# jenkinsm13/julia-spira

Hardware: AMD Instinct MI355X
Metric: Msamples/sec at 1920x1080 spp=64 depth=8; fraction of HBM roofline (higher is better)
Workload: dtype f64

## Files before the change

### julia-spira_amd/csrc/spira_device.h

```cpp
#pragma once
#include <hip/hip_runtime.h>
#include <stdint.h>
#include <type_traits>
#include "spira_fastdiv.h"

namespace spira {

__device__ __forceinline__ float sqrt_rn(float x) { return __builtin_sqrtf(x); }
__device__ __forceinline__ double sqrt_rn(double x) { return __builtin_sqrt(x); }

constexpr int kBlock = 256;
#ifndef SPIRA_WAVES_F32
#define SPIRA_WAVES_F32 5
#endif
#ifndef SPIRA_WAVES_F64
#define SPIRA_WAVES_F64 4
#endif
#define SPIRA_WAVES_PER_SIMD(T) (sizeof(T) == 8 ? SPIRA_WAVES_F64 : SPIRA_WAVES_F32)
constexpr uint32_t kMaxTries = 64;

template <class T> struct Vec { T x, y, z; };

template <class T> __device__ __forceinline__ Vec<T> mk(T x, T y, T z) { Vec<T> r; r.x = x; r.y = y; r.z = z; return r; }
template <class T> __device__ __forceinline__ Vec<T> operator+(Vec<T> a, Vec<T> b) { return mk<T>(a.x + b.x, a.y + b.y, a.z + b.z); }
// ... 1168 lines not shown
        a.blk_stats[4 * wid + 1] = n_rmw;
        a.blk_stats[4 * wid + 2] = n_store;
        a.blk_stats[4 * wid + 3] = FIRST ? 0u : n_seg;
    }
}

template <class T> struct PathArgs {
    SceneGlobal<T> scene;
    RenderConst<T> rc;
    RayQueue<T> q[2];
    uint32_t *qref[2];
    uint2 *qkey[2];
    uint32_t cam_consts;
    Pack3<T> *L;
    uint32_t *blk_stats;
    uint32_t cap;
    uint32_t pass;
    uint32_t n_first;
    uint32_t dense_pct;
    Pack4<T> *mesh_list;
    uint32_t mesh_min_batch;
    uint32_t refill_free;
    uint32_t mesh_mode;
    uint32_t *mesh_count;
    uint32_t resume_k, resume_nw;
    uint32_t *redo;
    uint32_t redo_only;
    Stats *stats;
    Pack4<T> *accum;
    FastDiv fd_keff;
    uint32_t k_eff;
    uint32_t accum_first;
    uint32_t l_private;
};

#ifndef SPIRA_RESOLVE_RUN
#define SPIRA_RESOLVE_RUN 4
#endif
__device__ __forceinline__ uint32_t owned_pixel(uint32_t w, uint32_t nw, uint32_t l) {
    constexpr uint32_t kRun = SPIRA_RESOLVE_RUN;
    static_assert(64 % kRun == 0, "a run length divides the wave");
    return ((l / kRun) * nw + w) * kRun + l % kRun;
}

template <class T>
__device__ __forceinline__ void resolve_pixel(Pack4<T> *accum, const Pack3<T> *L, uint32_t tile_pixels, uint32_t k_eff, bool first_pass, uint32_t p) {
    Pack4<T> acc;
    if (first_pass) { acc.x = 0; acc.y = 0; acc.z = 0; acc.w = 0; } else acc = accum[p];
    uint32_t s = 0;
    for (; s + 8 <= k_eff; s += 8) {
        Pack3<T> l[8];
#pragma unroll
        for (int k = 0; k < 8; ++k) l[k] = L[(size_t)(s + k) * tile_pixels + p];
#pragma unroll
        for (int k = 0; k < 8; ++k) { acc.x = acc.x + l[k].x; acc.y = acc.y + l[k].y; acc.z = acc.z + l[k].z; }
    }
    for (; s < k_eff; ++s) {
        const Pack3<T> l = L[(size_t)s * tile_pixels + p];
        acc.x = acc.x + l.x; acc.y = acc.y + l.y; acc.z = acc.z + l.z;
    }
    accum[p] = acc;
}
template <class T>
__device__ __forceinline__ void resolve_pixel_run(Pack4<T> *accum, const Pack3<T> *Lp, uint32_t k_eff, bool first_pass, uint32_t p) {
    constexpr uint32_t kRun = SPIRA_RESOLVE_RUN;
    Pack4<T> acc;
    if (first_pass) { acc.x = 0; acc.y = 0; acc.z = 0; acc.w = 0; } else acc = accum[p];
    uint32_t s = 0;
    for (; s + 8 <= k_eff; s += 8) {
        Pack3<T> l[8];
#pragma unroll
        for (int k = 0; k < 8; ++k) l[k] = Lp[(s + k) * kRun];
#pragma unroll
        for (int k = 0; k < 8; ++k) { acc.x = acc.x + l[k].x; acc.y = acc.y + l[k].y; acc.z = acc.z + l[k].z; }
    }
    for (; s < k_eff; ++s) {
        const Pack3<T> l = Lp[s * kRun];
        acc.x = acc.x + l.x; acc.y = acc.y + l.y; acc.z = acc.z + l.z;
    }
    accum[p] = acc;
}

__device__ __forceinline__ float pack_qref(uint32_t q, uint32_t, float) { return __uint_as_float(q); }
__device__ __forceinline__ double pack_qref(uint32_t q, uint32_t ref, double) { return __longlong_as_double((long long)((unsigned long long)q | ((unsigned long long)ref << 32))); }
__device__ __forceinline__ uint32_t unpack_q(float w) { return __float_as_uint(w); }
__device__ __forceinline__ uint32_t unpack_q(double w) { return (uint32_t)(unsigned long long)__double_as_longlong(w); }
__device__ __forceinline__ uint32_t unpack_ref(double w) { return (uint32_t)((unsigned long long)__double_as_longlong(w) >> 32); }

#ifdef SPIRA_MESH_STATS
__device__ unsigned long long g_mesh_dbg[32];
#define MESH_STAT(...) __VA_ARGS__
#else
#define MESH_STAT(...)
#endif

#ifndef SPIRA_CARRY_KEY
#define SPIRA_CARRY_KEY 1
#endif
#ifndef SPIRA_WAVES_B_F32
#define SPIRA_WAVES_B_F32 4
#endif
#ifndef SPIRA_WAVES_B_F64
#define SPIRA_WAVES_B_F64 SPIRA_WAVES_F64
#endif
#ifndef SPIRA_WAVES_PATH_F32
#define SPIRA_WAVES_PATH_F32 6
#endif
template <class T, int R, bool BVH, bool EXT, bool SPEC, int MODE = 0, bool TRI = true>
__global__ __launch_bounds__(kBlock, MODE == 2 ? (sizeof(T) == 8 ? SPIRA_WAVES_B_F64 : SPIRA_WAVES_B_F32) : (sizeof(T) == 4 ? SPIRA_WAVES_PATH_F32 : SPIRA_WAVES_F64)) void k_path(const PathArgs<T> a) {
    extern __shared__ __attribute__((aligned(32))) unsigned char lds_raw[];
    constexpr uint32_t WPB = kBlock / 64, SUB = 64 * R;
    constexpr bool kRefArray = sizeof(T) == 4;
    constexpr bool kCarry = SPIRA_CARRY_KEY && !BVH && !EXT;
    constexpr uint32_t kStageShift = 25, kRefMask = (1u << kStageShift) - 1u;
    const uint32_t lane = threadIdx.x & 63, wave = threadIdx.x >> 6;
    const uint32_t NW = gridDim.x * WPB, wid = blockIdx.x * WPB + wave;
    const RenderConst<T> &rc = a.rc;
    using Pol = typename std::conditional<SPEC, SpecDiv, ExactDiv>::type;
    Pol pol;
    if (!SPEC && a.redo_only) {
        uint32_t any = 0;
        for (uint32_t w = 0; w < WPB; ++w) any |= a.redo[blockIdx.x * WPB + w];
        if (!any) return;
    }
    T *cam_lds = reinterpret_cast<T *>(lds_raw + scene_lds_bytes<T>(a.scene.n_spheres, a.scene.n_materials, a.scene.n_triangles) + WPB * SUB * sizeof(Pack4<T>));
    if (threadIdx.x < 12) {
        const Vec<T> *cv = threadIdx.x < 3 ? &rc.cam_origin : (threadIdx.x < 6 ? &rc.cam_llc : (threadIdx.x < 9 ? &rc.cam_hor : &rc.cam_ver));
        const uint32_t cc = threadIdx.x % 3;
        cam_lds[threadIdx.x] = cc == 0 ? cv->x : (cc == 1 ? cv->y : cv->z);
    }
    Pack4<T> *cam_sph = reinterpret_cast<Pack4<T> *>(reinterpret_cast<unsigned char *>(cam_lds) + 128);
    constexpr bool kCam = !EXT;
    if (kCam && MODE != 2 && a.cam_consts)
        for (uint32_t i = threadIdx.x; i < a.scene.n_spheres; i += blockDim.x) {
            const T *sp = a.scene.spheres5 + 5 * (size_t)i;
            const Vec<T> oc = rc.cam_origin - mk<T>(sp[0], sp[1], sp[2]);
            Pack4<T> k; k.x = oc.x; k.y = oc.y; k.z = oc.z; k.w = dot(oc, oc) - sp[3] * sp[3];
            cam_sph[i] = k;
        }
    const SceneLds<T> sc = stage_scene<T>(a.scene, lds_raw);
    const PixelDiv<T> pix_div = pixel_divisors<T>(rc);
    if (!SPEC && a.redo_only) {
        if (!a.redo[wid]) return;
        if (lane == 0) atomicAdd(&a.stats->redone_waves, 1ull);
    }
    Pack4<T> *s_rnd = reinterpret_cast<Pack4<T> *>(lds_raw + scene_lds_bytes<T>(a.scene.n_spheres, a.scene.n_materials, a.scene.n_triangles)) + wave * SUB;
    constexpr uint32_t mesh_mode = BVH ? (uint32_t)MODE : 0u;
    const uint32_t kseg = mesh_mode == 2u ? a.resume_k : 1u;
    if (mesh_mode == 2u && wid * kseg >= a.resume_nw) return;
    const uint32_t region = wid * kseg * a.cap;
    const unsigned long long lt_mask = (1ull << lane) - 1ull;
    const uint32_t ref_base = sc.n_spheres + sc.n_triangles;
    const bool mixed = mesh_mode != 0u || rc.max_depth <= 128u;
    const uint32_t dense_pct = mixed ? a.dense_pct : 0u;
    const bool defer = mesh_mode != 0u || (BVH && mixed && a.mesh_list != nullptr);
    Pack4<T> *mlist = a.mesh_list + 3 * (size_t)region;
    uint32_t n_rmw = 0, n_store = 0, n_seg = 0, n_enq = 0, n_park = 0;
    uint32_t n_wtrips = 0, n_ltrips = 0;
    uint32_t n_in = 0;
    const bool own = !BVH && !EXT && !TRI && sizeof(T) == 8 && a.accum != nullptr;
    const uint32_t n_own = own ? 64u * a.k_eff : 0u;
    const uint32_t n_sub_first = own ? (n_own + SUB - 1) / SUB : (a.n_first + SUB - 1) / SUB;
    const bool priv = kCarry && own && a.l_private != 0;
    const uint32_t l_base = priv ? wid * n_own : 0u;

    auto park = [&](uint32_t slot_i, const Vec<T> o_, const Vec<T> d_, const Vec<T> beta_, T closest_, uint32_t q_, int prim_, uint32_t stage_hit) {
        Pack4<T> A, B, C;
        A.x = o_.x; A.y = o_.y; A.z = o_.z; A.w = d_.x;
        B.x = d_.y; B.y = d_.z; B.z = beta_.x; B.w = beta_.y;
        C.x = beta_.z; C.y = closest_; C.z = Bits<T>::from_u32(q_); C.w = Bits<T>::from_u32((uint32_t)(prim_ + 1) | (stage_hit << kStageShift));
        mlist[3 * (size_t)slot_i] = A; mlist[3 * (size_t)slot_i + 1] = B; mlist[3 * (size_t)slot_i + 2] = C;
    };
    uint32_t mfill = 0;
    constexpr int kMaxSeg = 16;
    uint32_t pfx[kMaxSeg + 1];
    bool segmented = false;
    {
        uint32_t cnt = 0;
        if (mesh_mode == 2u && lane < kseg && wid * kseg + lane < a.resume_nw) cnt = a.mesh_count[wid * kseg + lane];
        pfx[0] = 0;
#pragma unroll
        for (int j = 0; j < kMaxSeg; ++j) pfx[j + 1] = pfx[j] + (uint32_t)__builtin_amdgcn_readlane((int)cnt, j);
        if (mesh_mode == 2u) { mfill = pfx[kMaxSeg]; segmented = true; }
    }
    const uint32_t first_sub = own ? 0u : (mesh_mode == 1u ? (wid % a.resume_k) * (NW / a.resume_k) + wid / a.resume_k : wid);
    const uint32_t sub_step = own ? 1u : NW;
    MESH_STAT(unsigned long long dbg_t0 = __builtin_readcyclecounter(); unsigned long long dbg_sess = 0, dbg_walk = 0; uint32_t dbg_ns = 0, dbg_ws = 0, dbg_ls = 0, dbg_rf = 0, dbg_rays = 0, dbg_rounds = 0, dbg_ws1 = 0, dbg_ls1 = 0, dbg_h[4] = {0, 0, 0, 0};)
    for (uint32_t round = 0; ; ++round) {
        MESH_STAT(++dbg_rounds;)
        const bool first = mesh_mode != 2u && round == 0;
        const RayQueue<T> qin = a.q[(round + 1) & 1], qout = a.q[round & 1];
        const uint32_t *rin = a.qref[(round + 1) & 1];
        uint32_t *rout = a.qref[round & 1];
        const uint2 *kin = a.qkey[(round + 1) & 1];
        uint2 *kout = a.qkey[round & 1];
        const uint32_t limit = first ? (own ? n_own : a.n_first) : n_in;
        const uint32_t n_sub = first ? n_sub_first : (n_in + SUB - 1) / SUB;
        uint32_t fill = 0;
        for (uint32_t sub = first ? first_sub : 0u; sub < n_sub; sub += first ? sub_step : 1u) {
            Vec<T> o[R], beta[R];
            Pending<T> pend[R];
            ExtState<T> ex[R];
            uint32_t q[R], ent[R], stg[R], ref[R];
            uint32_t ka[R], kb[R];
            bool valid[R];
#pragma unroll
            for (int r = 0; r < R; ++r) {
                const uint32_t idx = sub * SUB + r * 64 + lane;
                valid[r] = false; stg[r] = round; ref[r] = 0; q[r] = 0; ka[r] = 0; kb[r] = 0;
                pend[r].kind = kDead; pend[r].rough = 0; pend[r].v = mk<T>(0, 0, 0);
                o[r] = mk<T>(0, 0, 0); beta[r] = mk<T>(1, 1, 1);
                bool parked = false; T park_t = 0; int park_prim = -1;
                uint32_t qf = idx;
                bool in = idx < limit;
                if (own && first) {
                    const uint32_t t = idx / SPIRA_RESOLVE_RUN, run = fastdiv(t, a.fd_keff);
                    const uint32_t px = owned_pixel(wid, NW, run * SPIRA_RESOLVE_RUN + idx % SPIRA_RESOLVE_RUN);
                    qf = (t - run * a.k_eff) * rc.tile_pixels + px;
                    in = in && px < rc.tile_pixels;
                }
                const uint32_t ql = priv ? l_base + idx : qf;
                if (in) {
                    if (first) {
                        uint32_t pixel, sample, pi, pj;
                        Vec<T> d;
                        q[r] = ql;
                        path_of<T>(rc, qf, a.pass, pi, pj, pixel, sample);
                        if (kCarry) { ka[r] = mix32(rc.sA + pixel) ^ (sample << 8); kb[r] = mix32(rc.sB ^ pixel) + (sample << 8); }
                        camera_ray_lds<T>(rc, cam_lds, pix_div, pi, pj, pixel, sample, o[r], d, pol);
                        if (EXT) { ex[r].flags = rc.flags; if (rc.flags & kExtSpectral) beta[r] = ext_wavelength<T>(sc, rc.sA, rc.sB, pixel, sample, ex[r]); }
                        T t; uint32_t slot = 0;
                        int prim;
                        if (defer) {
                            if (kCam && a.cam_consts) closest_hit_local<T, Pol, TRI, true>(sc, o[r], d, (T)0.001, t, prim, pol, cam_sph);
                            else closest_hit_local<T, Pol, TRI>(sc, o[r], d, (T)0.001, t, prim, pol);
                            parked = mesh_box_hit<T>(sc, o[r], d, t);
                        } else if (kCam && !BVH && a.cam_consts) { closest_hit_local<T, Pol, TRI, true>(sc, o[r], d, (T)0.001, t, prim, pol, cam_sph); }
                        else prim = closest_hit<T, BVH, Pol, TRI>(sc, o[r], d, (T)0.001, t, slot, pol);
                        ++n_seg;
                        if (parked) { park_t = t; park_prim = prim; pend[r].v = d; }
                        else if (prim < 0) {
                            const Vec<T> c = sky_term_x<T, EXT>(d, beta[r], &ex[r]);
                            Pack3<T> l; l.x = c.x; l.y = c.y; l.z = c.z;
                            a.L[ql] = l;
                            ++n_store;
                        } else {
                            valid[r] = true;
                            o[r] = o[r] + d * t;
                            ref[r] = (BVH && prim >= (int)ref_base) ? ref_base + slot : (uint32_t)prim;
                            pend[r].v = d;
                        }
                    } else {
                        const Pack4<T> A = qin.A[region + idx], B = qin.B[region + idx];
                        const Pack2<T> C = qin.C[region + idx];
                        o[r] = mk<T>(A.x, A.y, A.z);
                        pend[r].v = mk<T>(A.w, B.x, B.y);
                        beta[r] = mk<T>(B.z, B.w, C.x);
                        q[r] = unpack_q(C.y);
                        uint32_t w;
                        if constexpr (kRefArray) w = rin[region + idx]; else w = unpack_ref(C.y);
                        if (mixed) { stg[r] = w >> kStageShift; ref[r] = w & kRefMask; } else ref[r] = w;
                        if (kCarry) { const uint2 k = kin[region + idx]; ka[r] = k.x; kb[r] = k.y; }
                        valid[r] = true;
                    }
                }
                if (defer && first) {
                    const unsigned long long mp = __ballot(parked);
                    if (parked) park(mfill + __popcll(mp & lt_mask), o[r], pend[r].v, beta[r], park_t, q[r], park_prim, 0u);
                    mfill += (uint32_t)__popcll(mp); n_park += (uint32_t)__popcll(mp);
                }
            }
            while (true) {
                uint32_t n_list = 0, n_valid = 0;
#pragma unroll
                for (int r = 0; r < R; ++r) {
                    bool want = false;
                    RngKey key;
                    const Vec<T> d = pend[r].v;
                    pend[r].kind = kDead;
                    if (valid[r]) {
                        uint32_t pixel = 0, sample = 0, pi, pj;
                        const bool scatter = stg[r] + 1 < rc.max_depth;
                        int prim = (int)ref[r]; uint32_t slot = 0;
                        if (BVH && ref[r] >= ref_base) { prim = (int)ref_base; slot = ref[r] - ref_base; }
                        const uint32_t qi = q[r] & 0x7FFFFFFFu;
                        const bool has_l = (q[r] >> 31) != 0;
                        if (EXT) {
                            path_of<T>(rc, qi, a.pass, pi, pj, pixel, sample);
                            ex[r].flags = rc.flags;
                            if (rc.flags & kExtSpectral) (void)ext_wavelength<T>(sc, rc.sA, rc.sB, pixel, sample, ex[r]);
                        }
                        Vec<T> contrib;
                        const bool has_contrib = shade_hit<T, BVH, EXT, Pol, TRI>(sc, o[r], d, prim, slot, beta[r], scatter, contrib, pend[r], &ex[r], pol);
                        if (has_contrib) {
                            Pack3<T> l; l.x = contrib.x; l.y = contrib.y; l.z = contrib.z;
                            if (has_l) { const Pack3<T> l0 = a.L[qi]; l.x = l0.x + contrib.x; l.y = l0.y + contrib.y; l.z = l0.z + contrib.z; ++n_rmw; }
// ... 319 lines not shown
                if (!__any(walking)) { if (__any(finished)) continue; break; }
                const bool more = next < mfill;
                MESH_STAT(++dbg_rf; const unsigned long long dbg_w0 = __builtin_readcyclecounter();)
                uint32_t n_now = (uint32_t)__popcll(__ballot(walking));
                while (true) {
                    ++n_wtrips; n_ltrips += n_now;
                    MESH_STAT(++dbg_ws; { const uint32_t nl = (uint32_t)__popcll(__ballot(walking)); dbg_ls += nl; if (segmented) { ++dbg_ws1; dbg_ls1 += nl; } ++dbg_h[nl <= 8 ? 0 : (nl <= 24 ? 1 : (nl <= 48 ? 2 : 3))]; })
                    if (walking && !bvh8_step<T, kLdsStack>(sc, wk, ry, o_, d_, (T)0.001, (int)ref_base, closest, prim, slot, lstack, stack, lane)) { walking = false; finished = true; }
                    const uint32_t n_walk = (uint32_t)__popcll(__ballot(walking));
                    n_now = n_walk;
                    if (n_walk == 0 || (more && 64u - n_walk >= a.refill_free)) break;
                }

                MESH_STAT(dbg_walk += __builtin_readcyclecounter() - dbg_w0;)
            }
            }
            mfill = 0;
            segmented = false;
            MESH_STAT(dbg_sess += __builtin_readcyclecounter() - dbg_s0;)
        }
        n_in = fill;
        n_enq += fill;
        if (n_in == 0 && (mfill == 0 || mesh_mode == 1u)) break;
        __builtin_amdgcn_fence(__ATOMIC_RELEASE, "workgroup");
        __builtin_amdgcn_fence(__ATOMIC_ACQUIRE, "workgroup");
    }
    for (int sft = 32; sft > 0; sft >>= 1) { n_rmw += __shfl_down(n_rmw, sft); n_seg += __shfl_down(n_seg, sft); n_store += __shfl_down(n_store, sft); }
    const bool again = SPEC && __any(outside_window<T>(pol));
    if (own && !again && !(SPEC && a.redo_only == 2u)) {
        __builtin_amdgcn_fence(__ATOMIC_RELEASE, "workgroup");
        __builtin_amdgcn_fence(__ATOMIC_ACQUIRE, "workgroup");
        const uint32_t px = owned_pixel(wid, NW, lane);
        if (px < rc.tile_pixels) {
            if (priv) resolve_pixel_run<T>(a.accum, a.L + l_base + (lane / SPIRA_RESOLVE_RUN) * a.k_eff * SPIRA_RESOLVE_RUN + lane % SPIRA_RESOLVE_RUN, a.k_eff, a.accum_first != 0, px);
            else resolve_pixel<T>(a.accum, a.L, rc.tile_pixels, a.k_eff, a.accum_first != 0, px);
        }
        const uint32_t seg = __shfl(n_seg, 0), rmw = __shfl(n_rmw, 0), sto = __shfl(n_store, 0);
        if (lane < 4) {
            unsigned long long *f = lane == 0 ? &a.stats->segments : (lane == 1 ? &a.stats->rays_enqueued : (lane == 2 ? &a.stats->radiance_rmw : &a.stats->radiance_store));
            atomicAdd(f, (unsigned long long)(lane == 0 ? seg : (lane == 1 ? n_enq : (lane == 2 ? rmw : sto))));
        }
    }
    MESH_STAT(if (lane == 0) { unsigned long long *g = g_mesh_dbg + (mesh_mode == 2u ? 16 : 0);
                               atomicAdd(&g[0], __builtin_readcyclecounter() - dbg_t0); atomicAdd(&g[1], dbg_sess); atomicAdd(&g[2], (unsigned long long)dbg_ns);
                               atomicAdd(&g[3], (unsigned long long)dbg_ws); atomicAdd(&g[4], (unsigned long long)dbg_ls); atomicAdd(&g[5], (unsigned long long)dbg_rf);
                               atomicAdd(&g[6], (unsigned long long)dbg_rays); atomicAdd(&g[7], (unsigned long long)dbg_rounds); atomicAdd(&g[9], dbg_walk); atomicAdd(&g[10], 1ull); atomicAdd(&g[11], (unsigned long long)dbg_ws1); atomicAdd(&g[12], (unsigned long long)dbg_ls1);
                               atomicAdd(&g[8], (unsigned long long)dbg_h[0]); atomicAdd(&g[13], (unsigned long long)dbg_h[1]); atomicAdd(&g[14], (unsigned long long)dbg_h[2]); atomicAdd(&g[15], (unsigned long long)dbg_h[3]); })
    if (lane == 0) {
        if (mesh_mode == 2u) {
            const uint32_t row = 4 * wid * kseg;
            a.blk_stats[row] += n_seg; a.blk_stats[row + 1] += n_rmw; a.blk_stats[row + 2] += n_store; a.blk_stats[row + 3] += n_enq;
        } else {
            a.blk_stats[4 * wid] = n_seg;
            a.blk_stats[4 * wid + 1] = n_rmw;
            a.blk_stats[4 * wid + 2] = n_store;
            a.blk_stats[4 * wid + 3] = n_enq;
            if (mesh_mode == 1u) a.mesh_count[wid] = mfill;
        }
        if (SPEC) a.redo[wid] = again ? 1u : 0u;
        if (BVH && n_park && !again && !(SPEC && a.redo_only == 2u)) atomicAdd(&a.stats->rays_parked, (unsigned long long)n_park);
        if (BVH && mesh_mode != 1u && n_wtrips && !again && !(SPEC && a.redo_only == 2u)) { atomicAdd(&a.stats->mesh_wave_trips, (unsigned long long)n_wtrips); atomicAdd(&a.stats->mesh_lane_trips, (unsigned long long)n_ltrips); }
    }
}

template <class T, bool BVH, bool EXT>
__global__ __launch_bounds__(kBlock) void k_mega(const BounceArgs<T> a) {
    extern __shared__ __attribute__((aligned(32))) unsigned char lds_raw[];
// ... 813 lines not shown
```

### julia-spira_amd/csrc/spira_hip.hip

```cpp
#include <hip/hip_runtime.h>
#include <sys/mman.h>
#include <rccl/rccl.h>
#include <dlfcn.h>

#include <algorithm>
#include <atomic>
#include <chrono>
#include <cmath>
#include <cstdio>
#include <cstdlib>
#include <cstring>
#include <condition_variable>
#include <mutex>
#include <new>
#include <string>
#include <thread>
#include <vector>

#include "../../include/spira_hip.h"
#include "../../include/spira_spd.h"
#include "spira_device.h"
#include "spira_bvh.h"
#include "spira_validate.h"
#include "spira_plan.h"
// ... 534 lines not shown
        static_assert(SPIRA_SPD_N == spira::kSpdN && SPIRA_SPD_ROWS == spira::kSpdRows, "SPD table shape");
        T host[SPIRA_SPD_ROWS * SPIRA_SPD_N];
        for (int r = 0; r < SPIRA_SPD_ROWS; ++r)
            for (int i = 0; i < SPIRA_SPD_N; ++i) host[r * SPIRA_SPD_N + i] = (T)spira_spd_table[r][i];
        if (int rc = b.ensure(sizeof host)) return rc;
        HIP_TRY(hipMemcpy(b.p, host, sizeof host, hipMemcpyHostToDevice));
    }
    (void)st;
    g.spd = (const T *)b.p;
    return 0;
}

template <class T>
int check_handle(const spira_scene *h) {
    if (!h || h->magic != kSceneMagic) return fail(SPIRA_E_INVALID, "scene handle is NULL or was destroyed");
    if (h->prec != (int)sizeof(T)) return fail(SPIRA_E_INVALID, "scene handle was created in the other precision");
    if (h->device != tl_device) return fail(SPIRA_E_INVALID, "scene handle belongs to another device (spira_set_device)");
    return 0;
}

spira::Knobs read_knobs() {
    spira::Knobs k;
    k.batch_rays = env_u32("SPIRA_BATCH_RAYS", k.batch_rays);
    k.R = env_u32("SPIRA_R", k.R);
    k.blocks_per_cu = env_u32("SPIRA_BLOCKS_PER_CU", 0);
    k.defer_mesh = env_u32("SPIRA_DEFER_MESH", 1); k.mesh_two_pass = env_u32("SPIRA_MESH_TWO_PASS", 1);
    k.fused_resolve = env_u32("SPIRA_FUSED_RESOLVE", 1); k.private_l = env_u32("SPIRA_PRIVATE_L", 1);
    k.spec_div = env_u32("SPIRA_SPEC_DIV", 1);
    k.dense_pct = std::min<uint32_t>(env_u32("SPIRA_DENSE_PCT", 70), 100);
    k.mesh_min_batch = std::max<uint32_t>(1, env_u32("SPIRA_MESH_MIN_BATCH", 128));
    k.mesh_refill = std::min<uint32_t>(64, std::max<uint32_t>(1, env_u32("SPIRA_MESH_REFILL", 16)));
    k.mesh_fat_waves_per_cu = env_u32("SPIRA_MESH_FAT_WAVES_PER_CU", 16);
    k.cam_consts = env_u32("SPIRA_CAM_CONSTS", 1);
    return k;
}
template <class T>
spira::PlanIn plan_input(const Ctx &c, const spira_params *p, uint32_t rows, uint32_t nt_scene, bool progressive, bool caller_rng, bool out_on_device) {
    spira::PlanIn in;
    in.width = p->width; in.rows = rows; in.spp = p->spp; in.max_depth = p->max_depth; in.flags = p->flags; in.batch_rays = p->batch_rays;
    in.n_triangles = nt_scene; in.num_cus = (uint32_t)c.num_cus;
    in.progressive = progressive; in.caller_rng = caller_rng; in.out_on_device = out_on_device;
    in.prec = sizeof(T); in.block = spira::kBlock; in.waves_per_simd = SPIRA_WAVES_PER_SIMD(T); in.carry_key = SPIRA_CARRY_KEY;
    in.pack4 = sizeof(spira::Pack4<T>); in.pack3 = sizeof(spira::Pack3<T>); in.pack2 = sizeof(spira::Pack2<T>);
    in.k = read_knobs();
    return in;
}

int ensure_workspaces(Ctx &c, const spira::Workspace &w) {
    for (int i = 0; i < 2; ++i) {
        if (int rc = c.qA[i].ensure(w.queue4)) return rc;
        if (int rc = c.qB[i].ensure(w.queue4)) return rc;
        if (int rc = c.qC[i].ensure(w.queue2)) return rc;
        if (int rc = c.qR[i].ensure(w.q_ref)) return rc;
        if (int rc = c.qK[i].ensure(w.q_key)) return rc;
        if (int rc = c.qX[i].ensure(w.q_x)) return rc;
    }
    const struct { DevBuf &b; uint64_t bytes; } rest[] = {
        {c.mesh_list, w.mesh_list}, {c.mesh_count, w.mesh_count}, {c.redo, w.redo}, {c.blkstats, w.blkstats}, {c.L, w.L}, {c.counts, w.counts},
        {c.stats, sizeof(spira::Stats)}, {c.accum, w.accum}, {c.out_tmp, w.out_tmp}, {c.rng, w.rng},
        {c.hyb_state, w.hyb_state}, {c.hyb_mat, w.hyb_mat}, {c.hyb_flags, w.hyb_flags}};
    for (const auto &r : rest)
        if (int rc = r.b.ensure(r.bytes)) return rc;
    return 0;
}

template <class T>
int verify_path_args(const Ctx &c, const spira::PathArgs<T> &a, uint32_t first_launch_blocks) {
    using P4 = spira::Pack4<T>;
    using P2 = spira::Pack2<T>;
    spira::PathLaunch l;
    l.blocks = first_launch_blocks; l.cap = a.cap; l.n_first = a.n_first; l.k_eff = a.k_eff;
    l.tile_pixels = a.rc.tile_pixels; l.max_depth = a.rc.max_depth; l.flags = a.rc.flags; l.n_lds_triangles = a.scene.n_triangles;
    l.mesh_mode = a.mesh_mode; l.resume_k = a.resume_k; l.resume_nw = a.resume_nw;
    l.mesh = a.scene.n_bvh_tris != 0; l.pixel_owning = a.accum != nullptr; l.l_private = a.l_private != 0;
    l.prec = sizeof(T); l.wpb = spira::kBlock / 64; l.carry_key = SPIRA_CARRY_KEY;
    const spira::PathNeed need = spira::path_need(l);
    const uint64_t nw = need.nw, n = need.packets;
    auto covers = [](const DevBuf &b, const void *ptr, uint64_t bytes) { return ptr == b.p && b.p != nullptr && b.cap >= bytes; };
    const char *bad = need.fits ? nullptr : "the pass does not fit its queue regions";
    if (a.rc.max_depth > 1 || l.mesh)
        for (int i = 0; i < 2 && !bad; ++i) {
            if (!covers(c.qA[i], a.q[i].A, n * sizeof(P4)) || !covers(c.qB[i], a.q[i].B, n * sizeof(P4)) || !covers(c.qC[i], a.q[i].C, n * sizeof(P2))) bad = "hit queues";
            else if (sizeof(T) == 4 && !covers(c.qR[i], a.qref[i], n * sizeof(uint32_t))) bad = "hit reference arrays";
            else if (!l.mesh && !covers(c.qK[i], a.qkey[i], n * sizeof(uint2))) bad = "carried RNG keys";
        }
    if (!bad && a.mesh_list && !covers(c.mesh_list, a.mesh_list, 3 * n * sizeof(P4))) bad = "mesh lists";
    if (!bad && a.mesh_mode != 0 && (!a.mesh_list || !covers(c.mesh_count, a.mesh_count, nw * sizeof(uint32_t)) || !need.resume_ok)) bad = "parked-ray counts of a two-launch mesh pass";
    if (!bad && a.redo && !covers(c.redo, a.redo, nw * sizeof(uint32_t))) bad = "redo flags";
    if (!bad && !covers(c.blkstats, a.blk_stats, nw * 4 * sizeof(uint32_t))) bad = "per-wave statistics";
    if (!bad && !covers(c.L, a.L, need.l_entries * sizeof(spira::Pack3<T>))) bad = "per-path radiance";
    if (!bad && !covers(c.stats, a.stats, sizeof(spira::Stats))) bad = "counters";
    if (!bad && a.accum && (!covers(c.accum, a.accum, (uint64_t)a.rc.tile_pixels * sizeof(P4)) || !need.owning_ok)) bad = "pixel-owning pass";
    if (!bad && a.l_private && !need.private_ok) bad = "wave-private radiance blocks";
    if (bad) return fail(SPIRA_E_LIMIT, std::string("internal: a workspace is smaller than the launch needs (") + bad + ")");
    return 0;
}

template <class T>
int validate_call(const spira_scene *h, const T *spheres5, const T *materials8, const T *triangles10, const T *camera12, const spira_params *p,
                  const T *out_hdr, const T *out_img, bool progressive, uint32_t sample0, const uint32_t *rng_states, uint32_t *rows) {
    if (!p) return fail(SPIRA_E_INVALID, "params is NULL");
    const uint32_t nt = triangles10 ? p->n_triangles : 0;
    if (h) { if (int rc = check_handle<T>(h)) return rc; }
    else if (int rc = validate_scene<T>(spheres5, materials8, triangles10, p->n_spheres, p->n_materials, nt)) return rc;
    if (int rc = validate_params(camera12, p, h ? h->store.nt : nt, rows)) return rc;
    if (!out_hdr && !out_img) return fail(SPIRA_E_INVALID, "both outputs are NULL");
    const char *msg = nullptr;
    if (int rc = spira::sample_range_check(progressive, sample0, p->spp, &msg)) return fail(rc, msg);
    if (progressive && (p->flags & SPIRA_SEM_MASK) == SPIRA_SEM_HYBRID) return fail(SPIRA_E_UNSUPPORTED, "SPIRA_SEM_HYBRID has no accumulate entry (its image is a mean of tone-mapped samples)");
    if (progressive && (p->flags & SPIRA_SEM_MASK) == SPIRA_SEM_METAL && sample0 > 0 && !rng_states)
        return fail(SPIRA_E_INVALID, "SPIRA_SEM_METAL with sample0 > 0 needs rng_states (the LCG states the previous call left); "
                                     "without them every call would replay the samples of the first");
    return 0;
}

template <class T> struct Call {
    Ctx &c;
    hipStream_t st;
    const spira_params *p;
    const spira::Plan &plan;
    spira::BounceArgs<T> a{};
    size_t lds = 0;
    int spec = 0;
    bool progressive = false, profile = false;
    uint32_t sample0 = 0, *d_rng = nullptr;
    uint64_t launches = 0, metal_launches = 0;
// ... 93 lines not shown
    const dim3 grid(k.plan.blocks(k.a.n_first));
    const bool ext = (k.p->flags & (SPIRA_EXT_DIELECTRIC | SPIRA_EXT_SPECTRAL)) != 0;
    if (k.a.scene.n_bvh_tris) { if (ext) launch_lds(spira::k_mega<T, true, true>, grid, k.block(), k.lds, k.st, k.a); else launch_lds(spira::k_mega<T, true, false>, grid, k.block(), k.lds, k.st, k.a); }
    else { if (ext) launch_lds(spira::k_mega<T, false, true>, grid, k.block(), k.lds, k.st, k.a); else launch_lds(spira::k_mega<T, false, false>, grid, k.block(), k.lds, k.st, k.a); }
    ++k.launches;
    return 0;
}

template <class T>
int enqueue_path_pass(Call<T> &k, uint32_t *stat_rows) {
    using P4 = typename Call<T>::P4;
    Ctx &c = k.c;
    const spira::Plan &plan = k.plan;
    const spira::Knobs &kn = plan.in.k;
    spira::PathArgs<T> pa{};
    pa.scene = k.a.scene; pa.rc = k.a.rc; pa.L = k.a.L; pa.pass = k.a.pass; pa.n_first = k.a.n_first;
    pa.dense_pct = kn.dense_pct;
    pa.mesh_list = plan.defer_mesh ? (P4 *)c.mesh_list.p : nullptr;
    const spira::Geometry g = plan.geometry(pa.n_first);
    const uint32_t G = g.G;
    pa.cap = g.cap;
    *stat_rows = G * plan.wpb;
    for (int i = 0; i < 2; ++i) {
        pa.q[i] = k.queue(i);
        pa.qref[i] = (uint32_t *)c.qR[i].p;
        pa.qkey[i] = (uint2 *)c.qK[i].p;
    }
    pa.blk_stats = (uint32_t *)c.blkstats.p;
    pa.stats = k.stats();
    if (k.spec) pa.redo = k.redo();
    pa.mesh_mode = 0; pa.mesh_count = nullptr; pa.resume_k = 1; pa.resume_nw = 0;
    pa.mesh_min_batch = kn.mesh_min_batch;
    pa.refill_free = kn.mesh_refill;
    size_t lds_a = k.lds + (size_t)plan.wpb * plan.sub * sizeof(P4) + 128;
    pa.cam_consts = (kn.cam_consts && pa.scene.n_spheres && lds_a + (size_t)pa.scene.n_spheres * sizeof(P4) <= (size_t)160 * 1024) ? 1u : 0u;
    if (pa.cam_consts) lds_a += (size_t)pa.scene.n_spheres * sizeof(P4);
    if (plan.two_pass) {
        pa.mesh_mode = 1; pa.mesh_count = (uint32_t *)c.mesh_count.p;
        pa.resume_nw = G * plan.wpb; pa.resume_k = plan.fat_k(pa.resume_nw);
    }
    if (plan.fused) {
        pa.accum = k.accum(); pa.k_eff = plan.k_eff(pa.pass); pa.fd_keff = spira::fastdiv_make(pa.k_eff);
        pa.accum_first = (pa.pass == 0 && !k.progressive) ? 1u : 0u;
        pa.l_private = plan.l_private ? 1u : 0u;
    }
    if (int rc = verify_path_args<T>(c, pa, G)) return rc;
    HIP_TRY(hipEventRecord(c.ev_pool[c.ev_used++], k.st));
    if (int rc = launch_path<T>((int)plan.R, dim3(G), lds_a, k.st, pa, k.spec)) return rc;
    if (int rc = lds_optin_failed()) return rc;
    k.launches += k.spec ? 2 : 1;
    if (pa.mesh_mode == 1) {
        if (c.ev_mid.size() <= c.ev_mid_used) {
            hipEvent_t e;
            HIP_TRY(hipEventCreate(&e));
            c.ev_mid.push_back(e); c.ev_mid_end.push_back(0);
        }
        HIP_TRY(hipEventRecord(c.ev_mid[c.ev_mid_used], k.st));
        c.ev_mid_end[c.ev_mid_used++] = c.ev_used;
        spira::PathArgs<T> pb = pa;
        pb.mesh_mode = 2; pb.n_first = 0;
        const uint32_t nwb = pa.resume_nw / pa.resume_k;
        launch_path_resume_entry<T>((int)plan.R, dim3((nwb + plan.wpb - 1) / plan.wpb), lds_a, k.st, pb);
        if (int rc = lds_optin_failed()) return rc;
        ++k.launches;
    }
    HIP_TRY(hipEventRecord(c.ev_pool[c.ev_used++], k.st));
    return 0;
}

template <class T>
int enqueue_bounce_pass(Call<T> &k, uint32_t *stat_rows) {
    using P4 = typename Call<T>::P4;
    Ctx &c = k.c;
    const spira::Plan &plan = k.plan;
    const spira::Geometry g = plan.geometry(k.a.n_first);
    const size_t nw = (size_t)g.G * plan.wpb;
    k.a.cap = g.cap;
// ... 1249 lines not shown
```

### julia-spira_amd/csrc/spira_plan.h

```cpp
#pragma once
#include <algorithm>
#include <cstdint>

#include "../../include/spira_hip.h"

namespace spira {

struct Knobs {
    uint32_t batch_rays = 160u << 20;
    uint32_t R = 2;
    uint32_t blocks_per_cu = 0;
    uint32_t defer_mesh = 1, mesh_two_pass = 1, fused_resolve = 1, private_l = 1;
    uint32_t spec_div = 1;
    uint32_t dense_pct = 70, mesh_min_batch = 128, mesh_refill = 16, mesh_fat_waves_per_cu = 16, cam_consts = 1;
};

struct PlanIn {
    uint32_t width = 0, rows = 0;
    uint32_t spp = 0, max_depth = 0, flags = 0, batch_rays = 0;
    uint32_t n_triangles = 0;
    uint32_t num_cus = 0;
    bool progressive = false, caller_rng = false, out_on_device = false;
    bool adaptive = false;
    uint32_t prec = 0, block = 0, waves_per_simd = 0, carry_key = 0;
    uint32_t pack4 = 0, pack3 = 0, pack2 = 0;
    Knobs k;
};

enum class Org { Black, Hybrid, MetalWavefront, Metal, Cpu, Mega, Path, Bounce };

struct Geometry { uint32_t G, cap; };

struct Workspace {
    uint64_t queue4 = 0, queue2 = 0, q_ref = 0, q_key = 0, q_x = 0;
    uint64_t mesh_list = 0, mesh_count = 0, redo = 0, blkstats = 0, L = 0, counts = 0, accum = 0, out_tmp = 0, rng = 0;
    uint64_t hyb_state = 0, hyb_mat = 0, hyb_flags = 0;
};

struct Plan {
    PlanIn in;
    Org org = Org::Black;
    uint32_t R = 2, wpb = 0, sub = 0, max_blocks = 0;
    uint64_t tile_pixels = 0, batch = 0;
    uint32_t slots = 0, n_pass = 0;
    bool mesh_scene = false, defer_mesh = false, two_pass = false;
    bool fused = false, l_private = false;
    bool spec_allowed = false;
    uint32_t G_max = 0, cap_max = 0;
    uint64_t q_rays = 0;
    uint32_t ppw = 0, G_metal = 0;
    Workspace ws;

    Geometry geometry(uint64_t n_first) const {
        if (fused) {
            const uint64_t k = n_first / tile_pixels;
            return {(uint32_t)((tile_pixels + 64 * wpb - 1) / (64 * wpb)), (uint32_t)((64 * k + sub - 1) / sub * sub)};
        }
        const uint64_t n_sub = (n_first + sub - 1) / sub;
        const uint32_t G = (uint32_t)std::min<uint64_t>((n_sub + wpb - 1) / wpb, max_blocks);
        const uint64_t nw = (uint64_t)G * wpb;
        return {G, (uint32_t)(((n_sub + nw - 1) / nw) * sub)};
    }
    uint32_t k_eff(uint32_t pass) const { return std::min(slots, in.spp - pass * slots); }
    uint32_t n_first(uint32_t pass) const { return (uint32_t)((uint64_t)k_eff(pass) * tile_pixels); }
    uint32_t blocks(uint64_t n) const { return (uint32_t)std::min<uint64_t>((n + in.block - 1) / in.block, max_blocks); }
    uint32_t fat_k(uint32_t nw) const {
        const uint32_t fat = std::max<uint32_t>(1, in.num_cus * in.k.mesh_fat_waves_per_cu);
        uint32_t k = 16;
        while (k > 1 && (nw % k != 0 || nw / k < fat)) k >>= 1;
        return k;
    }
    int spec(bool moderate) const {
        uint32_t s = spec_allowed ? in.k.spec_div : 0;
        if (s == 1 && !moderate) s = 0;
        return s > 2 ? 1 : (int)s;
    }
};

inline int sample_range_check(bool progressive, uint32_t sample0, uint32_t spp, const char **msg) {
    if (progressive && (uint64_t)sample0 + spp > SPIRA_MAX_SPP) { *msg = "sample0 + spp exceeds 2^24"; return SPIRA_E_LIMIT; }
    return 0;
}

inline int make_plan(const PlanIn &in, Plan &pl, const char **msg) {
    auto bad = [&](const char *m) { *msg = m; return SPIRA_E_LIMIT; };
    pl = Plan{};
    pl.in = in;
    const Knobs &k = in.k;
    const uint32_t sem = in.flags & SPIRA_SEM_MASK, kern = in.flags & SPIRA_KERNEL_MASK;
    const bool ext = (in.flags & (SPIRA_EXT_DIELECTRIC | SPIRA_EXT_SPECTRAL)) != 0;
    const uint64_t tp = pl.tile_pixels = (uint64_t)in.rows * in.width;
    const uint32_t target = in.batch_rays ? in.batch_rays : k.batch_rays;
    uint64_t slots = std::min<uint64_t>(std::max<uint64_t>(1, target / tp), in.spp);
    const uint64_t n_pass = (in.spp + slots - 1) / slots;
    slots = (in.spp + n_pass - 1) / n_pass;
    if (slots * tp > 0x7FFFFFFFull) return bad("tile too large: rows*width must be < 2^31");
    pl.slots = (uint32_t)slots;
// ... 42 lines not shown
        w.queue4 = n * in.pack4; w.queue2 = n * in.pack2; w.q_x = n * 2 * sizeof(uint32_t); w.L = n * in.pack3;
        if (!in.caller_rng) w.rng = tp * sizeof(uint32_t);
        w.blkstats = nw * stat_row; w.redo = nw * redo_per_wave;
        break;
    }
    case Org::Metal: case Org::Cpu: case Org::Mega:
        w.L = pl.batch * in.pack3; w.blkstats = waves * stat_row;
        w.redo = (pl.org == Org::Metal ? pl.blocks(tp) : pl.org == Org::Cpu ? pl.max_blocks : 0) * (uint64_t)pl.wpb * redo_per_wave;
        break;
    case Org::Bounce:
        if (in.max_depth > 1) { w.queue4 = pl.q_rays * in.pack4; w.queue2 = pl.q_rays * in.pack2; }
        w.L = pl.batch * in.pack3;
        w.counts = (uint64_t)(in.max_depth + 2) * waves * sizeof(uint32_t); w.blkstats = (uint64_t)(in.max_depth + 1) * waves * stat_row;
        break;
    case Org::Path:
        if (in.max_depth > 1 || pl.mesh_scene) {
            w.queue4 = pl.q_rays * in.pack4; w.queue2 = pl.q_rays * in.pack2;
            if (in.prec == 4) w.q_ref = pl.q_rays * sizeof(uint32_t);
            if (!pl.defer_mesh) w.q_key = pl.q_rays * 2 * sizeof(uint32_t);
        }
        if (pl.defer_mesh) w.mesh_list = 3 * pl.q_rays * in.pack4;
        if (pl.two_pass) w.mesh_count = waves * sizeof(uint32_t);
        w.redo = waves * redo_per_wave; w.blkstats = waves * stat_row;
        w.L = (pl.l_private ? std::max<uint64_t>(pl.batch, 64ull * waves * pl.slots) : pl.batch) * in.pack3;
        break;
    }
    return 0;
}

struct PathLaunch {
    uint32_t blocks = 0, cap = 0, n_first = 0, k_eff = 0;
    uint32_t tile_pixels = 0, max_depth = 0, flags = 0, n_lds_triangles = 0;
    uint32_t mesh_mode = 0, resume_k = 1, resume_nw = 0;
    bool mesh = false, pixel_owning = false, l_private = false;
    uint32_t prec = 0, wpb = 0, carry_key = 0;
};
struct PathNeed {
    uint64_t nw, packets, l_entries;
    bool fits, resume_ok, owning_ok, private_ok;
};
inline PathNeed path_need(const PathLaunch &a) {
    PathNeed n{};
    n.nw = (uint64_t)a.blocks * a.wpb;
    n.packets = n.nw * a.cap;
    n.fits = a.n_first <= n.packets;
    n.resume_ok = a.resume_k != 0 && a.resume_k <= 16 && n.nw % a.resume_k == 0 && a.resume_nw == n.nw;
    n.l_entries = a.l_private ? std::max<uint64_t>(a.n_first, 64ull * n.nw * a.k_eff) : a.n_first;
    const uint64_t tp = a.tile_pixels;
    n.owning_ok = a.prec == 8 && !a.n_lds_triangles && !a.mesh && !(a.flags & (SPIRA_EXT_DIELECTRIC | SPIRA_EXT_SPECTRAL)) && a.k_eff != 0 && a.k_eff <= 64 &&
                  (uint64_t)a.k_eff * tp == a.n_first && 64 * n.nw >= tp && a.cap >= 64ull * a.k_eff;
    n.private_ok = a.pixel_owning && a.carry_key && a.max_depth <= 128 && n.l_entries <= 0x80000000ull;
    return n;
}

struct AdaptiveIn {
    uint32_t min_spp = 0, batch_spp = 0, spp = 0;
    double tolerance = 0, floor = 0;
    uint64_t tile_pixels = 0;
    uint32_t prec = 0, pack3 = 0, num_cus = 0;
};
constexpr uint32_t kAdaptiveItems = 256, kAdaptiveWpb = 4;
struct AdaptiveRound { uint32_t samples, chunk, ppw, grid; uint64_t waves; };
struct AdaptivePlan {
    AdaptiveIn in;
    uint32_t levels = 0;
    uint64_t list_cap = 0;
    uint64_t list_bytes = 0, q_bytes = 0, n_bytes = 0, count_bytes = 0;
    uint64_t lds_round = 0;
    uint32_t level(uint32_t r) const { return (uint32_t)std::min<uint64_t>((uint64_t)in.min_spp + (uint64_t)r * in.batch_spp, in.spp); }
    AdaptiveRound round(uint32_t r, uint64_t n_active) const {
        AdaptiveRound a{};
        a.samples = level(r) - level(r - 1);
        a.chunk = std::min(a.samples, kAdaptiveItems);
        const uint64_t want_waves = std::max<uint64_t>(1, (uint64_t)in.num_cus * 16);
        const uint64_t spread = (n_active + want_waves - 1) / want_waves;
        a.ppw = (uint32_t)std::max<uint64_t>(1, std::min<uint64_t>(std::min<uint32_t>(64, kAdaptiveItems / a.chunk), spread));
        a.waves = (n_active + a.ppw - 1) / a.ppw;
        a.grid = (uint32_t)((a.waves + kAdaptiveWpb - 1) / kAdaptiveWpb);
        return a;
    }
};
inline int adaptive_check(uint32_t min_spp, uint32_t batch_spp, uint32_t spp, double tolerance, double floor, const char **msg) {
    if (min_spp < 2) { *msg = "spira_adaptive: min_spp must be >= 2 (a variance needs two samples)"; return SPIRA_E_INVALID; }
    if (batch_spp < 1) { *msg = "spira_adaptive: batch_spp must be >= 1"; return SPIRA_E_INVALID; }
// ... 85 lines not shown
```

Before: 27600.

## Accumulate first-hit sky radiance in per-wave LDS prefix sums instead of global L

When an entire wave's primary rays miss geometry and the run is next in order, the sky terms go to LDS scratch. They are then folded into per-pixel running sums in LDS rather than written to the global radiance buffer. The fused resolve starts from these prefix sums and skips the already-summed samples, which cuts HBM writes and reads for sky-only primary samples. In exchange it adds extra LDS per wave, wave-level syncs and ballots in the hot loop, plus planner and validation plumbing.

Result: no change. 27630 (median of 2 runs) (+0.1%).

```diff
diff --git a/julia-spira_amd/csrc/spira_device.h b/julia-spira_amd/csrc/spira_device.h
--- a/julia-spira_amd/csrc/spira_device.h
+++ b/julia-spira_amd/csrc/spira_device.h
@@ -1224,7 +1224,10 @@
     uint32_t k_eff;
     uint32_t accum_first;
     uint32_t l_private;
+    uint32_t sky_prefix;
 };
+constexpr uint32_t kSkyPrefixSums = 64 * 3, kSkyPrefixRuns = 64 / 4;
+template <class T> constexpr uint32_t sky_prefix_bytes() { return kSkyPrefixSums * (uint32_t)sizeof(T) + kSkyPrefixRuns * (uint32_t)sizeof(uint32_t); }
 
 #ifndef SPIRA_RESOLVE_RUN
 #define SPIRA_RESOLVE_RUN 4
@@ -1254,11 +1257,12 @@
     accum[p] = acc;
 }
 template <class T>
-__device__ __forceinline__ void resolve_pixel_run(Pack4<T> *accum, const Pack3<T> *Lp, uint32_t k_eff, bool first_pass, uint32_t p) {
+__device__ __forceinline__ void resolve_pixel_run(Pack4<T> *accum, const Pack3<T> *Lp, uint32_t k_eff, bool first_pass, uint32_t p, uint32_t s0 = 0, const T *sum0 = nullptr) {
     constexpr uint32_t kRun = SPIRA_RESOLVE_RUN;
     Pack4<T> acc;
     if (first_pass) { acc.x = 0; acc.y = 0; acc.z = 0; acc.w = 0; } else acc = accum[p];
-    uint32_t s = 0;
+    if (s0) { acc.x = sum0[0]; acc.y = sum0[1]; acc.z = sum0[2]; }
+    uint32_t s = s0;
     for (; s + 8 <= k_eff; s += 8) {
         Pack3<T> l[8];
 #pragma unroll
@@ -1271,6 +1275,20 @@
         acc.x = acc.x + l.x; acc.y = acc.y + l.y; acc.z = acc.z + l.z;
     }
     accum[p] = acc;
+}
+
+__device__ __forceinline__ uint32_t local_copy(uint32_t v) { asm volatile("" : "+v"(v)); return v; }
+template <class T>
+__device__ __forceinline__ void sky_prefix_add(T *sum, const T *term, uint32_t i, bool start, bool first_pass, const Pack4<T> *accum, uint32_t px) {
+    constexpr uint32_t kRun = SPIRA_RESOLVE_RUN;
+    const uint32_t c = i % 3, pp = i / 3;
+    T acc;
+    if (!start) acc = sum[i];
+    else if (first_pass) acc = 0;
+    else acc = reinterpret_cast<const T *>(&accum[px])[c];
+#pragma unroll
+    for (uint32_t s = 0; s < 64 / kRun; ++s) acc = acc + term[(s * kRun + pp) * 3 + c];
+    sum[i] = acc;
 }
 
 __device__ __forceinline__ float pack_qref(uint32_t q, uint32_t, float) { return __uint_as_float(q); }
@@ -1305,7 +1323,8 @@
     constexpr bool kRefArray = sizeof(T) == 4;
     constexpr bool kCarry = SPIRA_CARRY_KEY && !BVH && !EXT;
     constexpr uint32_t kStageShift = 25, kRefMask = (1u << kStageShift) - 1u;
-    const uint32_t lane = threadIdx.x & 63, wave = threadIdx.x >> 6;
+    constexpr bool kScalarWave = !BVH && !EXT && !TRI && sizeof(T) == 8;
+    const uint32_t lane = threadIdx.x & 63, wave = kScalarWave ? (uint32_t)__builtin_amdgcn_readfirstlane((int)(threadIdx.x >> 6)) : threadIdx.x >> 6;
     const uint32_t NW = gridDim.x * WPB, wid = blockIdx.x * WPB + wave;
     const RenderConst<T> &rc = a.rc;
     using Pol = typename std::conditional<SPEC, SpecDiv, ExactDiv>::type;
@@ -1350,11 +1369,19 @@
     uint32_t n_rmw = 0, n_store = 0, n_seg = 0, n_enq = 0, n_park = 0;
     uint32_t n_wtrips = 0, n_ltrips = 0;
     uint32_t n_in = 0;
-    const bool own = !BVH && !EXT && !TRI && sizeof(T) == 8 && a.accum != nullptr;
+    constexpr bool kOwnable = !BVH && !EXT && !TRI && sizeof(T) == 8;
+    const bool own = kOwnable && a.accum != nullptr;
     const uint32_t n_own = own ? 64u * a.k_eff : 0u;
     const uint32_t n_sub_first = own ? (n_own + SUB - 1) / SUB : (a.n_first + SUB - 1) / SUB;
     const bool priv = kCarry && own && a.l_private != 0;
     const uint32_t l_base = priv ? wid * n_own : 0u;
+    const bool skyp = kOwnable && priv && a.sky_prefix != 0;
+    const uint32_t pfx_off = kOwnable ? (uint32_t)__builtin_amdgcn_readfirstlane((int)(wave * sky_prefix_bytes<T>())) + (a.cam_consts ? a.scene.n_spheres * (uint32_t)sizeof(Pack4<T>) : 0u) : 0u;
+    T *pfx_sum = reinterpret_cast<T *>(reinterpret_cast<unsigned char *>(cam_sph) + pfx_off);
+    uint32_t *pfx_cnt = reinterpret_cast<uint32_t *>(pfx_sum + kSkyPrefixSums);
+    if constexpr (kOwnable) {
+        if (skyp && lane < kSkyPrefixRuns) pfx_cnt[lane] = 0;
+    }
 
     auto park = [&](uint32_t slot_i, const Vec<T> o_, const Vec<T> d_, const Vec<T> beta_, T closest_, uint32_t q_, int prim_, uint32_t stage_hit) {
         Pack4<T> A, B, C;
@@ -1405,6 +1432,7 @@
                 bool parked = false; T park_t = 0; int park_prim = -1;
                 uint32_t qf = idx;
                 bool in = idx < limit;
+                bool hold = false;
                 if (own && first) {
                     const uint32_t t = idx / SPIRA_RESOLVE_RUN, run = fastdiv(t, a.fd_keff);
                     const uint32_t px = owned_pixel(wid, NW, run * SPIRA_RESOLVE_RUN + idx % SPIRA_RESOLVE_RUN);
@@ -1430,11 +1458,22 @@
                         } else if (kCam && !BVH && a.cam_consts) { closest_hit_local<T, Pol, TRI, true>(sc, o[r], d, (T)0.001, t, prim, pol, cam_sph); }
                         else prim = closest_hit<T, BVH, Pol, TRI>(sc, o[r], d, (T)0.001, t, slot, pol);
                         ++n_seg;
+                        if constexpr (kOwnable) {
+                            if (skyp) {
+                                constexpr uint32_t kRun = SPIRA_RESOLVE_RUN;
+                                const uint32_t t0 = (sub * SUB + r * 64) / kRun, run = fastdiv(t0, a.fd_keff), j = (t0 - run * a.k_eff) / (64 / kRun);
+                                hold = __ballot(prim < 0 && pfx_cnt[run] == j) == ~0ull;
+                            }
+                        }
                         if (parked) { park_t = t; park_prim = prim; pend[r].v = d; }
                         else if (prim < 0) {
                             const Vec<T> c = sky_term_x<T, EXT>(d, beta[r], &ex[r]);
                             Pack3<T> l; l.x = c.x; l.y = c.y; l.z = c.z;
-                            a.L[ql] = l;
+                            if (kOwnable && hold) {
+                                T *term = reinterpret_cast<T *>(s_rnd) + local_copy(lane) * 3;
+                                term[0] = l.x; term[1] = l.y; term[2] = l.z;
+                            }
+                            else a.L[ql] = l;
                             ++n_store;
                         } else {
                             valid[r] = true;
@@ -1454,6 +1493,18 @@
                         if (mixed) { stg[r] = w >> kStageShift; ref[r] = w & kRefMask; } else ref[r] = w;
                         if (kCarry) { const uint2 k = kin[region + idx]; ka[r] = k.x; kb[r] = k.y; }
                         valid[r] = true;
+                    }
+                }
+                if constexpr (kOwnable) {
+                    if (hold) {
+                        constexpr uint32_t kRun = SPIRA_RESOLVE_RUN;
+                        const uint32_t t0 = (sub * SUB + r * 64) / kRun, run = fastdiv(t0, a.fd_keff), j = (t0 - run * a.k_eff) / (64 / kRun);
+                        const T *term = reinterpret_cast<const T *>(s_rnd);
+                        wave_lds_sync();
+                        const uint32_t i = local_copy(lane);
+                        if (i < 3 * kRun) sky_prefix_add<T>(pfx_sum + run * kRun * 3, term, i, j == 0, a.accum_first != 0, a.accum, owned_pixel(wid, NW, run * kRun + i / 3));
+                        if (i == 0) pfx_cnt[run] = j + 1;
+                        wave_lds_sync();
                     }
                 }
                 if (defer && first) {
@@ -1839,7 +1890,9 @@
         __builtin_amdgcn_fence(__ATOMIC_ACQUIRE, "workgroup");
         const uint32_t px = owned_pixel(wid, NW, lane);
         if (px < rc.tile_pixels) {
-            if (priv) resolve_pixel_run<T>(a.accum, a.L + l_base + (lane / SPIRA_RESOLVE_RUN) * a.k_eff * SPIRA_RESOLVE_RUN + lane % SPIRA_RESOLVE_RUN, a.k_eff, a.accum_first != 0, px);
+            if (kOwnable && skyp) resolve_pixel_run<T>(a.accum, a.L + l_base + (lane / SPIRA_RESOLVE_RUN) * a.k_eff * SPIRA_RESOLVE_RUN + lane % SPIRA_RESOLVE_RUN, a.k_eff, a.accum_first != 0, px,
+                                                       pfx_cnt[lane / SPIRA_RESOLVE_RUN] * (64 / SPIRA_RESOLVE_RUN), pfx_sum + lane * 3);
+            else if (priv) resolve_pixel_run<T>(a.accum, a.L + l_base + (lane / SPIRA_RESOLVE_RUN) * a.k_eff * SPIRA_RESOLVE_RUN + lane % SPIRA_RESOLVE_RUN, a.k_eff, a.accum_first != 0, px);
             else resolve_pixel<T>(a.accum, a.L, rc.tile_pixels, a.k_eff, a.accum_first != 0, px);
         }
         const uint32_t seg = __shfl(n_seg, 0), rmw = __shfl(n_rmw, 0), sto = __shfl(n_store, 0);
diff --git a/julia-spira_amd/csrc/spira_hip.hip b/julia-spira_amd/csrc/spira_hip.hip
--- a/julia-spira_amd/csrc/spira_hip.hip
+++ b/julia-spira_amd/csrc/spira_hip.hip
@@ -590,6 +590,7 @@
     k.mesh_refill = std::min<uint32_t>(64, std::max<uint32_t>(1, env_u32("SPIRA_MESH_REFILL", 16)));
     k.mesh_fat_waves_per_cu = env_u32("SPIRA_MESH_FAT_WAVES_PER_CU", 16);
     k.cam_consts = env_u32("SPIRA_CAM_CONSTS", 1);
+    k.sky_prefix = env_u32("SPIRA_SKY_PREFIX", 1);
     return k;
 }
 template <class T>
@@ -630,7 +631,7 @@
     l.blocks = first_launch_blocks; l.cap = a.cap; l.n_first = a.n_first; l.k_eff = a.k_eff;
     l.tile_pixels = a.rc.tile_pixels; l.max_depth = a.rc.max_depth; l.flags = a.rc.flags; l.n_lds_triangles = a.scene.n_triangles;
     l.mesh_mode = a.mesh_mode; l.resume_k = a.resume_k; l.resume_nw = a.resume_nw;
-    l.mesh = a.scene.n_bvh_tris != 0; l.pixel_owning = a.accum != nullptr; l.l_private = a.l_private != 0;
+    l.mesh = a.scene.n_bvh_tris != 0; l.pixel_owning = a.accum != nullptr; l.l_private = a.l_private != 0; l.sky_prefix = a.sky_prefix != 0;
     l.prec = sizeof(T); l.wpb = spira::kBlock / 64; l.carry_key = SPIRA_CARRY_KEY;
     const spira::PathNeed need = spira::path_need(l);
     const uint64_t nw = need.nw, n = need.packets;
@@ -650,6 +651,7 @@
     if (!bad && !covers(c.stats, a.stats, sizeof(spira::Stats))) bad = "counters";
     if (!bad && a.accum && (!covers(c.accum, a.accum, (uint64_t)a.rc.tile_pixels * sizeof(P4)) || !need.owning_ok)) bad = "pixel-owning pass";
     if (!bad && a.l_private && !need.private_ok) bad = "wave-private radiance blocks";
+    if (!bad && a.sky_prefix && !need.sky_ok) bad = "sky prefix rows";
     if (bad) return fail(SPIRA_E_LIMIT, std::string("internal: a workspace is smaller than the launch needs (") + bad + ")");
     return 0;
 }
@@ -809,9 +811,10 @@
     pa.mesh_mode = 0; pa.mesh_count = nullptr; pa.resume_k = 1; pa.resume_nw = 0;
     pa.mesh_min_batch = kn.mesh_min_batch;
     pa.refill_free = kn.mesh_refill;
-    size_t lds_a = k.lds + (size_t)plan.wpb * plan.sub * sizeof(P4) + 128;
-    pa.cam_consts = (kn.cam_consts && pa.scene.n_spheres && lds_a + (size_t)pa.scene.n_spheres * sizeof(P4) <= (size_t)160 * 1024) ? 1u : 0u;
-    if (pa.cam_consts) lds_a += (size_t)pa.scene.n_spheres * sizeof(P4);
+    static_assert(sizeof(P4) == 4 * sizeof(T), "Plan::path_lds sizes the work lists with PlanIn::pack4");
+    const spira::PathLds lds_plan = plan.path_lds(k.lds, pa.scene.n_spheres, pa.pass);
+    const size_t lds_a = (size_t)lds_plan.bytes;
+    pa.cam_consts = lds_plan.cam_consts ? 1u : 0u;
     if (plan.two_pass) {
         pa.mesh_mode = 1; pa.mesh_count = (uint32_t *)c.mesh_count.p;
         pa.resume_nw = G * plan.wpb; pa.resume_k = plan.fat_k(pa.resume_nw);
@@ -820,6 +823,8 @@
         pa.accum = k.accum(); pa.k_eff = plan.k_eff(pa.pass); pa.fd_keff = spira::fastdiv_make(pa.k_eff);
         pa.accum_first = (pa.pass == 0 && !k.progressive) ? 1u : 0u;
         pa.l_private = plan.l_private ? 1u : 0u;
+        pa.sky_prefix = lds_plan.sky_prefix ? 1u : 0u;
+        static_assert(sizeof(T) != 8 || spira::sky_prefix_bytes<T>() == 64 * 3 * sizeof(T) + 16 * sizeof(uint32_t), "Plan::sky_prefix_lds");
     }
     if (int rc = verify_path_args<T>(c, pa, G)) return rc;
     HIP_TRY(hipEventRecord(c.ev_pool[c.ev_used++], k.st));
diff --git a/julia-spira_amd/csrc/spira_plan.h b/julia-spira_amd/csrc/spira_plan.h
--- a/julia-spira_amd/csrc/spira_plan.h
+++ b/julia-spira_amd/csrc/spira_plan.h
@@ -13,6 +13,7 @@
     uint32_t defer_mesh = 1, mesh_two_pass = 1, fused_resolve = 1, private_l = 1;
     uint32_t spec_div = 1;
     uint32_t dense_pct = 70, mesh_min_batch = 128, mesh_refill = 16, mesh_fat_waves_per_cu = 16, cam_consts = 1;
+    uint32_t sky_prefix = 1;
 };
 
 struct PlanIn {
@@ -30,6 +31,8 @@
 enum class Org { Black, Hybrid, MetalWavefront, Metal, Cpu, Mega, Path, Bounce };
 
 struct Geometry { uint32_t G, cap; };
+struct PathLds { uint64_t bytes; bool cam_consts, sky_prefix; };
+constexpr uint64_t kLdsPerWorkgroup = 160 * 1024;
 
 struct Workspace {
     uint64_t queue4 = 0, queue2 = 0, q_ref = 0, q_key = 0, q_x = 0;
@@ -63,6 +66,14 @@
     }
     uint32_t k_eff(uint32_t pass) const { return std::min(slots, in.spp - pass * slots); }
     uint32_t n_first(uint32_t pass) const { return (uint32_t)((uint64_t)k_eff(pass) * tile_pixels); }
+    bool sky_prefix(uint32_t pass) const { return fused && l_private && in.k.sky_prefix != 0 && k_eff(pass) % 16 == 0; }
+    uint64_t sky_prefix_lds(uint32_t pass) const { return sky_prefix(pass) ? (uint64_t)wpb * (64 * 3 * in.prec + 16 * sizeof(uint32_t)) : 0; }
+    PathLds path_lds(uint64_t scene_bytes, uint32_t n_spheres, uint32_t pass) const {
+        PathLds l{scene_bytes + (uint64_t)wpb * sub * in.pack4 + 128 + sky_prefix_lds(pass), false, sky_prefix(pass)};
+        l.cam_consts = in.k.cam_consts && n_spheres && l.bytes + (uint64_t)n_spheres * in.pack4 <= kLdsPerWorkgroup;
+        if (l.cam_consts) l.bytes += (uint64_t)n_spheres * in.pack4;
+        return l;
+    }
     uint32_t blocks(uint64_t n) const { return (uint32_t)std::min<uint64_t>((n + in.block - 1) / in.block, max_blocks); }
     uint32_t fat_k(uint32_t nw) const {
         const uint32_t fat = std::max<uint32_t>(1, in.num_cus * in.k.mesh_fat_waves_per_cu);
@@ -171,12 +182,12 @@
     uint32_t blocks = 0, cap = 0, n_first = 0, k_eff = 0;
     uint32_t tile_pixels = 0, max_depth = 0, flags = 0, n_lds_triangles = 0;
     uint32_t mesh_mode = 0, resume_k = 1, resume_nw = 0;
-    bool mesh = false, pixel_owning = false, l_private = false;
+    bool mesh = false, pixel_owning = false, l_private = false, sky_prefix = false;
     uint32_t prec = 0, wpb = 0, carry_key = 0;
 };
 struct PathNeed {
     uint64_t nw, packets, l_entries;
-    bool fits, resume_ok, owning_ok, private_ok;
+    bool fits, resume_ok, owning_ok, private_ok, sky_ok;
 };
 inline PathNeed path_need(const PathLaunch &a) {
     PathNeed n{};
@@ -189,6 +200,7 @@
     n.owning_ok = a.prec == 8 && !a.n_lds_triangles && !a.mesh && !(a.flags & (SPIRA_EXT_DIELECTRIC | SPIRA_EXT_SPECTRAL)) && a.k_eff != 0 && a.k_eff <= 64 &&
                   (uint64_t)a.k_eff * tp == a.n_first && 64 * n.nw >= tp && a.cap >= 64ull * a.k_eff;
     n.private_ok = a.pixel_owning && a.carry_key && a.max_depth <= 128 && n.l_entries <= 0x80000000ull;
+    n.sky_ok = a.pixel_owning && a.l_private && a.k_eff != 0 && a.k_eff % 16 == 0;
     return n;
 }
 
```
